# ksahlin/IsoCon

Hardware: AMD Instinct MI355X
Metric: read x candidate alignments/sec (NN-graph build, 50k x 2.5kb reads) (higher is better)
Workload: dtype u64; 1 GPU; C3: 50000 synthetic CCS reads (50000 unique), ~2500 bp, 10 isoforms, seed 30001; 1-set NN graph; edges=78526, graph_digest=65944c838d76a6c9, parallelism=single GPU

## Files before the change

isocon_amd/csrc/ed_lanes.hpp:

```cpp
#pragma once
#include "band_core.hpp"
#include "common.hpp"
#include "ed_lanes_core.hpp"
#include "nn.hpp"

namespace isocon {

template <bool NN>
__global__ __launch_bounds__(256) void k_ed_lanes(DevStore S, NNParams P, const uint32_t *__restrict__ pa, const uint32_t *__restrict__ pb,
                                                   const int32_t *__restrict__ pk, uint64_t n_pairs, int32_t *__restrict__ out,
                                                   const unsigned long long *__restrict__ live = nullptr)
{
    if (live != nullptr) { const uint64_t nl = *live; n_pairs = nl < n_pairs ? nl : n_pairs; }
    const uint64_t i = (uint64_t)blockIdx.x * 256u + threadIdx.x;
    uint32_t x = 0, y = 0;
    bool valid = i < n_pairs;
    if (valid) {
        x = pa[i]; y = pb[i];
        valid = x != 0xffffffffu && y != 0xffffffffu && x < S.n && y < S.n && (!NN || x != y);
        if (!valid) { x = 0; y = 0; }
    }
    const int32_t m = S.lens[x], n = S.lens[y];
    bool upd_x = false, upd_y = false;
    int32_t k = -1;
    if (NN) {
        upd_x = valid && P.qflag[x] && P.tflag[y];
        upd_y = valid && P.qflag[y] && P.tflag[x];
        int32_t kx = -1, ky = -1;
        if (upd_x) { const int32_t b = load_relaxed_agent(P.best + x); kx = b < m ? b : m; }
        if (upd_y) { const int32_t b = load_relaxed_agent(P.best + y); ky = b < n ? b : n; }
        k = kx > ky ? kx : ky;
        if (k > 63) k = 63;
    } else if (valid) {
        k = pk[i];
        if (k > 63) k = 63;
    }
    const int32_t d = m - n, ad = d < 0 ? -d : d;
    bool run = valid && k >= 0 && ad <= k;
    int32_t r = -1;
    if (run && (m == 0 || n == 0)) { r = ad; run = false; }
    const uint64_t *planes = S.planes;
    const uint32_t nseq = S.n;
    const int32_t nchunks = (int32_t)S.nchunks;
    auto x_lo = [&](int32_t ci) -> uint64_t { return ci < nchunks ? planes[((size_t)ci * nseq + x) * 2] : 0; };
    auto x_hi = [&](int32_t ci) -> uint64_t { return ci < nchunks ? planes[((size_t)ci * nseq + x) * 2 + 1] : 0; };
    auto y_lo = [&](int32_t ci) -> uint64_t { return ci < nchunks ? planes[((size_t)ci * nseq + y) * 2] : 0; };
    auto y_hi = [&](int32_t ci) -> uint64_t { return ci < nchunks ? planes[((size_t)ci * nseq + y) * 2 + 1] : 0; };
    const int32_t rd = lane_pair_distance(x_lo, x_hi, y_lo, y_hi, m, n, k, run, [](bool b) { return __ballot(b) != 0; });
    if (run) r = rd;
    if (!NN) {
        if (i < n_pairs) out[i] = r;
        return;
    }
    bool hit_x = false, hit_y = false;
    if (r >= P.min_d) {
        if (upd_x && r <= m) hit_x = nn_take(P, x, r);
        if (upd_y && r <= n) hit_y = nn_take(P, y, r);
    }
    nn_append(P, hit_x, (int32_t)x, (int32_t)y, r);
    nn_append(P, hit_y, (int32_t)y, (int32_t)x, r);
}

}
```

isocon_amd/csrc/ed_lanes_core.hpp:

```cpp
#pragma once
#include "band_core.hpp"

namespace isocon {

ISO_HD uint32_t funnel32(uint32_t hi, uint32_t lo, int s)
{
#if defined(__HIP_DEVICE_COMPILE__)
    return __builtin_amdgcn_alignbit(hi, lo, (uint32_t)s);
#else
    return s ? (lo >> s) | (hi << (32 - s)) : lo;
#endif
}

ISO_HD uint32_t splat_bit(uint32_t w, int j)
{
#if defined(__HIP_DEVICE_COMPILE__)
    return (uint32_t)__builtin_amdgcn_sbfe((int)w, (uint32_t)j, 1u);
#else
    return 0u - ((w >> j) & 1u);
#endif
}

ISO_HD uint32_t lane_valid32(int32_t o, int32_t m)
{
    int32_t lo = -o, hi = m - o;
    if (lo < 0) lo = 0;
    if (hi > 32) hi = 32;
    if (hi <= lo) return 0u;
    const uint32_t upto_hi = hi >= 32 ? 0xffffffffu : ((1u << hi) - 1u);
    return upto_hi & ~((1u << lo) - 1u);
}

template <class XL, class XH, class YL, class YH, class Any>
ISO_HD int32_t lane_pair_distance(XL x_lo, XH x_hi, YL y_lo, YH y_hi, int32_t m, int32_t n, int32_t k, bool run, Any any)
{
    const int32_t d = m - n;
    int32_t a0 = lane_emin(d, k < 0 ? 0 : k);
    if (a0 < -63) a0 = -63;
    const int32_t nv = -a0;
    int32_t bstar = d - a0;
    if (bstar < 0) bstar = 0;
    if (bstar > 63) bstar = 63;
    BandLane<1> L;
    band_init<1>(L, nv, bstar);
    int32_t r = -1;
    int32_t o = -nv;
    uint32_t L0, L1, L2, H0, H1, H2;
    {
        const uint64_t tl = ~stream64(x_lo, o), th = ~stream64(x_hi, o);
        L0 = (uint32_t)tl; L1 = (uint32_t)(tl >> 32); H0 = (uint32_t)th; H1 = (uint32_t)(th >> 32);
        L2 = (uint32_t)~stream64(x_lo, o + 64);
        H2 = (uint32_t)~stream64(x_hi, o + 64);
    }
    for (int32_t c0 = 0;; c0 += 32) {
        if (!any(run)) break;
        const uint32_t wl = (uint32_t)stream64(y_lo, c0), wh = (uint32_t)stream64(y_hi, c0);
        const bool full = c0 + 32 <= n;
        if (o >= 0 && !any(run && !full)) {
            uint32_t zreg = 0;
#if defined(__HIP_DEVICE_COMPILE__)
#pragma unroll
#endif
            for (int jj = 0; jj < 32; ++jj) {
                const uint32_t sl = splat_bit(wl, jj), sh = splat_bit(wh, jj);
                const uint32_t nl0 = funnel32(L1, L0, jj), nl1 = funnel32(L2, L1, jj), nh0 = funnel32(H1, H0, jj), nh1 = funnel32(H2, H1, jj);
#if defined(__HIP_DEVICE_COMPILE__)
                const uint32_t e0 = __builtin_amdgcn_bitop3_b32(nl0 ^ sl, nh0, sh, 0x60);
                const uint32_t e1 = __builtin_amdgcn_bitop3_b32(nl1 ^ sl, nh1, sh, 0x60);
#else
                const uint32_t e0 = (nl0 ^ sl) & (nh0 ^ sh), e1 = (nl1 ^ sl) & (nh1 ^ sh);
#endif
                band_step_eq64z(L.VP[0], L.VN[0], zreg, ((uint64_t)e1 << 32) | e0);
            }
#if defined(__HIP_DEVICE_COMPILE__)
            L.ztop += (uint32_t)__popc(zreg);
#else
            L.ztop += (uint32_t)__builtin_popcount(zreg);
#endif
        } else {
            const uint32_t V0 = lane_valid32(o, m), V1 = lane_valid32(o + 32, m), V2 = lane_valid32(o + 64, m);
#if defined(__HIP_DEVICE_COMPILE__)
#pragma unroll 1
#endif
            for (int jj = 0; jj < 32; ++jj) {
                if (run && c0 + jj < n) {
                    uint64_t NL[1], NH[1], VM[1];
                    NL[0] = ((uint64_t)funnel32(L2, L1, jj) << 32) | funnel32(L1, L0, jj);
                    NH[0] = ((uint64_t)funnel32(H2, H1, jj) << 32) | funnel32(H1, H0, jj);
                    VM[0] = ((uint64_t)funnel32(V2, V1, jj) << 32) | funnel32(V1, V0, jj);
                    band_step<1, true>(L, NL, NH, VM, splat_bit(wl, jj), splat_bit(wh, jj));
                }
            }
        }
        if (run) {
            const bool fin = c0 + 32 >= n;
            const int32_t dv = band_diag_value<1>(L, nv, fin ? n : c0 + 32);
            if (fin) { r = dv <= k ? dv : -1; run = false; }
            else if (dv > k) run = false;
        }
        o += 32;
        L0 = L1; L1 = L2; H0 = H1; H1 = H2;
        L2 = (uint32_t)~stream64(x_lo, o + 64);
        H2 = (uint32_t)~stream64(x_hi, o + 64);
    }
    return r;
}

}
```

Measured before the change: 84.45 billion alignments/s.

## Precompute per-block match masks in LDS table for banded edit-distance columns

For each 32-column block, each lane builds a 4-entry table in shared memory holding the match masks of the x window for each of the four nucleotides. Each column then fetches the matching record through an index packed from the y bits, with a small prefetch queue, and applies two funnel shifts. This replaces the per-column splat, four funnel shifts and two bitop3 operations. In exchange it adds LDS stores and loads, LDS space and scheduling barriers, so whether it helps depends on LDS latency versus the VALU ops removed.

```diff
diff --git a/isocon_amd/csrc/ed_lanes.hpp b/isocon_amd/csrc/ed_lanes.hpp
--- a/isocon_amd/csrc/ed_lanes.hpp
+++ b/isocon_amd/csrc/ed_lanes.hpp
@@ -46,7 +46,9 @@
     auto x_hi = [&](int32_t ci) -> uint64_t { return ci < nchunks ? planes[((size_t)ci * nseq + x) * 2 + 1] : 0; };
     auto y_lo = [&](int32_t ci) -> uint64_t { return ci < nchunks ? planes[((size_t)ci * nseq + y) * 2] : 0; };
     auto y_hi = [&](int32_t ci) -> uint64_t { return ci < nchunks ? planes[((size_t)ci * nseq + y) * 2 + 1] : 0; };
-    const int32_t rd = lane_pair_distance(x_lo, x_hi, y_lo, y_hi, m, n, k, run, [](bool b) { return __ballot(b) != 0; });
+    __shared__ eq_rec_t eq_tab[4 * EQ_TABLE_RECS];
+    const EqFromTable eq(eq_tab, threadIdx.x >> 6, threadIdx.x & 63u);
+    const int32_t rd = lane_pair_distance(x_lo, x_hi, y_lo, y_hi, m, n, k, run, [](bool b) { return __ballot(b) != 0; }, eq);
     if (run) r = rd;
     if (!NN) {
         if (i < n_pairs) out[i] = r;
diff --git a/isocon_amd/csrc/ed_lanes_core.hpp b/isocon_amd/csrc/ed_lanes_core.hpp
--- a/isocon_amd/csrc/ed_lanes_core.hpp
+++ b/isocon_amd/csrc/ed_lanes_core.hpp
@@ -31,8 +31,74 @@
     return upto_hi & ~((1u << lo) - 1u);
 }
 
-template <class XL, class XH, class YL, class YH, class Any>
-ISO_HD int32_t lane_pair_distance(XL x_lo, XH x_hi, YL y_lo, YH y_hi, int32_t m, int32_t n, int32_t k, bool run, Any any)
+struct EqFromPlanes {
+    uint32_t L0, L1, L2, H0, H1, H2, wl, wh;
+    ISO_HD void block(uint32_t l0, uint32_t l1, uint32_t l2, uint32_t h0, uint32_t h1, uint32_t h2, uint32_t tl, uint32_t th)
+    {
+        L0 = l0; L1 = l1; L2 = l2; H0 = h0; H1 = h1; H2 = h2; wl = tl; wh = th;
+    }
+    ISO_HD void column(int jj, uint32_t &e0, uint32_t &e1)
+    {
+        const uint32_t sl = splat_bit(wl, jj), sh = splat_bit(wh, jj);
+        const uint32_t nl0 = funnel32(L1, L0, jj), nl1 = funnel32(L2, L1, jj), nh0 = funnel32(H1, H0, jj), nh1 = funnel32(H2, H1, jj);
+#if defined(__HIP_DEVICE_COMPILE__)
+        e0 = __builtin_amdgcn_bitop3_b32(nl0 ^ sl, nh0, sh, 0x60);
+        e1 = __builtin_amdgcn_bitop3_b32(nl1 ^ sl, nh1, sh, 0x60);
+#else
+        e0 = (nl0 ^ sl) & (nh0 ^ sh);
+        e1 = (nl1 ^ sl) & (nh1 ^ sh);
+#endif
+    }
+};
+
+typedef uint32_t eq_rec_t __attribute__((vector_size(16)));
+enum { EQ_TABLE_LANES = 64, EQ_TABLE_RECS = 4 * EQ_TABLE_LANES , EQ_TABLE_AHEAD = 4 };
+
+struct EqFromTable {
+    eq_rec_t *tab;
+    uint32_t self;
+    uint32_t E, O;
+    eq_rec_t q[EQ_TABLE_AHEAD];
+    ISO_HD EqFromTable(eq_rec_t *table, uint32_t wave, uint32_t lane) : tab(table), self(wave * EQ_TABLE_RECS | lane), E(0), O(0) {}
+    ISO_HD uint32_t index(int jj) const
+    {
+        const uint32_t t = (jj & 1) ? (O >> (jj - 1)) & 3u : (E >> jj) & 3u;
+        return self | t * EQ_TABLE_LANES;
+    }
+    ISO_HD void block(uint32_t L0, uint32_t L1, uint32_t L2, uint32_t H0, uint32_t H1, uint32_t H2, uint32_t wl, uint32_t wh)
+    {
+#if defined(__HIP_DEVICE_COMPILE__)
+#pragma unroll
+#endif
+        for (uint32_t t = 0; t < 4; ++t) {
+            const uint32_t sl = 0u - (t & 1u), sh = 0u - (t >> 1);
+            const eq_rec_t rec = {(L0 ^ sl) & (H0 ^ sh), (L1 ^ sl) & (H1 ^ sh), (L2 ^ sl) & (H2 ^ sh), 0u};
+            tab[self | t * EQ_TABLE_LANES] = rec;
+        }
+        E = (wl & 0x55555555u) | ((wh & 0x55555555u) << 1);
+        O = ((wl >> 1) & 0x55555555u) | (wh & 0xAAAAAAAAu);
+#if defined(__HIP_DEVICE_COMPILE__)
+#pragma unroll
+#endif
+        for (int jj = 0; jj < EQ_TABLE_AHEAD; ++jj) q[jj] = tab[index(jj)];
+    }
+    ISO_HD void column(int jj, uint32_t &e0, uint32_t &e1)
+    {
+#if defined(__HIP_DEVICE_COMPILE__)
+        __builtin_amdgcn_sched_barrier(0);
+#endif
+        eq_rec_t rec = q[jj % EQ_TABLE_AHEAD];
+#if defined(__HIP_DEVICE_COMPILE__)
+        asm volatile("" : "+v"(rec));
+#endif
+        if (jj + EQ_TABLE_AHEAD < 32) q[jj % EQ_TABLE_AHEAD] = tab[index(jj + EQ_TABLE_AHEAD)];
+        e0 = funnel32(rec[1], rec[0], jj);
+        e1 = funnel32(rec[2], rec[1], jj);
+    }
+};
+
+template <class XL, class XH, class YL, class YH, class Any, class Eq = EqFromPlanes>
+ISO_HD int32_t lane_pair_distance(XL x_lo, XH x_hi, YL y_lo, YH y_hi, int32_t m, int32_t n, int32_t k, bool run, Any any, Eq eq = Eq())
 {
     const int32_t d = m - n;
     int32_t a0 = lane_emin(d, k < 0 ? 0 : k);
@@ -58,18 +124,13 @@
         const bool full = c0 + 32 <= n;
         if (o >= 0 && !any(run && !full)) {
             uint32_t zreg = 0;
+            eq.block(L0, L1, L2, H0, H1, H2, wl, wh);
 #if defined(__HIP_DEVICE_COMPILE__)
 #pragma unroll
 #endif
             for (int jj = 0; jj < 32; ++jj) {
-                const uint32_t sl = splat_bit(wl, jj), sh = splat_bit(wh, jj);
-                const uint32_t nl0 = funnel32(L1, L0, jj), nl1 = funnel32(L2, L1, jj), nh0 = funnel32(H1, H0, jj), nh1 = funnel32(H2, H1, jj);
-#if defined(__HIP_DEVICE_COMPILE__)
-                const uint32_t e0 = __builtin_amdgcn_bitop3_b32(nl0 ^ sl, nh0, sh, 0x60);
-                const uint32_t e1 = __builtin_amdgcn_bitop3_b32(nl1 ^ sl, nh1, sh, 0x60);
-#else
-                const uint32_t e0 = (nl0 ^ sl) & (nh0 ^ sh), e1 = (nl1 ^ sl) & (nh1 ^ sh);
-#endif
+                uint32_t e0, e1;
+                eq.column(jj, e0, e1);
                 band_step_eq64z(L.VP[0], L.VN[0], zreg, ((uint64_t)e1 << 32) | e0);
             }
 #if defined(__HIP_DEVICE_COMPILE__)
```

Result: faster. 88.46 billion alignments/s (median of 6 runs) (+4.8%).
